# lzzcd001/MeshDiffusion

Measured on AMD Instinct MI355X. Metric: denoise steps/sec on 64^3x4 DMTet grids (sample-steps/s = n_gpus*batch*steps/wall), higher is better.
Workload: dtype f16f6 in the Winograd convs behind a GroupNorm (fp16 hi*hi MFMA + MX block-scaled e2m3 cross terms in a K-concatenated scaled MFMA at twice the e4m3 rate; operands and weights equalised per input channel by a power of two: md_wino_equaliser, after the load-time calibration from the measured operand

## Files before the change

### include/meshdiffusion_hip.h

```cpp
#ifndef MESHDIFFUSION_HIP_H
#define MESHDIFFUSION_HIP_H

#include <stdint.h>

#ifdef __cplusplus
extern "C" {
#endif

#define MD_OK 0
#define MD_ERR_BAD_ARG (-1)
#define MD_ERR_UNSUPPORTED (-2)
#define MD_ERR_NO_DEVICE (-3)

#define MD_ABI_VERSION 16

enum {
  MD_CFG_C3_128 = 0,
  MD_CFG_C3_128_K16 = 1,
  MD_CFG_C3_32 = 2,
  MD_CFG_C3_LOW = 3,
  MD_CFG_C3_S2 = 4,
  MD_CFG_G1_128 = 5,
  MD_CFG_G1_128_LOW = 6,
  MD_CFG_G1_64_LOW = 7,
// ... 86 lines not shown
                           int32_t W, void* stream);
int md_ncdhw_to_s16b(const float* x, void* out, int32_t batch, int32_t C, int32_t c_pad,
                     int64_t P, void* stream);
int md_f32b_to_ncdhw(const float* x, float* out, int32_t batch, int32_t C, int64_t P, void* stream);
int md_ncdhw_to_f32b(const float* x, float* out, int32_t batch, int32_t C, int64_t P, void* stream);
int md_s16b_to_ncdhw(const void* x, float* out, int32_t batch, int32_t C, int64_t P, void* stream);

int md_softmax_keys(const float* s, void* p, int32_t batch, int32_t n_keys, int32_t n_q,
                    void* stream);

int md_nin_f32(const float* x1, const float* x2, int32_t c1, int32_t c2, const void* wpk, const float* bias,
               float* out, int32_t batch, int32_t cout, int64_t P, int32_t n_cu, void* stream);

int64_t md_wino_operand_bytes(int32_t batch, int32_t cin, int32_t D, int32_t H, int32_t W);
int md_wino_prep(const float* x1, const float* x2, int32_t c1, int32_t c2, const float* ac, int32_t silu, int32_t ups,
                 void* t_out, int32_t batch, int32_t D, int32_t H, int32_t W, float drop_p, uint64_t drop_seed, void* stream);
int64_t md_wino_weight_bytes(int32_t cout, int32_t cin);
int md_wino_pack_weights(const float* w, void* wpk, int32_t cout, int32_t cin, int64_t s_row, int64_t s_k, int32_t flip,
                         void* stream);
int md_conv3_wino(const void* t_in, const void* wpk, float* out, const float* bias, int64_t bias_bstride,
                  const float* residual, int64_t res_bstride, double* stats, int32_t batch, int32_t cin, int32_t cout,
                  int32_t D, int32_t H, int32_t W, int32_t variant, void* stream);

int md_wino_equaliser(const float* gamma, const float* beta, const float* w, int32_t cout, int32_t cin, int64_t s_row, int64_t s_k,
                      float* eq, void* stream);
int md_wino_equaliser_measured(const float* gamma, const float* beta, const float* w, const float* a2m, int32_t cout, int32_t cin,
                               int64_t s_row, int64_t s_k, float* eq, void* stream);
int md_wino_operand_ms(const float* x1, const float* x2, int32_t c1, int32_t c2, const float* ac, int32_t silu, int32_t batch, int64_t P,
                       float* ms, void* stream);
int md_wino_prep_f8(const float* x1, const float* x2, int32_t c1, int32_t c2, const float* ac, int32_t silu, int32_t ups,
                    const float* eq, void* t_out, int32_t batch, int32_t D, int32_t H, int32_t W, void* stream);
int64_t md_wino_weight_bytes_f8(int32_t cout, int32_t cin);
int md_wino_pack_weights_f8(const float* w, const float* eq, void* wpk, int32_t cout, int32_t cin, int64_t s_row, int64_t s_k, void* stream);
int md_conv3_wino_f8(const void* t_in, const void* wpk, float* out, const float* bias, int64_t bias_bstride,
                     const float* residual, int64_t res_bstride, double* stats, int32_t batch, int32_t cin, int32_t cout,
                     int32_t D, int32_t H, int32_t W, void* stream);
int md_absmax(const float* x, int64_t n, uint32_t* amax_bits, void* stream);
int md_wino_prep_dual_f6(const float* x, int32_t c, void* t_out, void* u_out, float* sums, float tscale, const uint32_t* amax_bits,
                         int32_t batch, int32_t D, int32_t H, int32_t W, void* stream);
int md_conv3_wino_f6_scaled(const void* t_in, const void* wpk, float* out, const float* bias, int64_t bias_bstride,
                            const float* residual, int64_t res_bstride, double* stats, int32_t batch, int32_t cin, int32_t cout,
                            int32_t D, int32_t H, int32_t W, float out_scale, const uint32_t* amax_bits, void* stream);

int md_wino_prep_f6(const float* x1, const float* x2, int32_t c1, int32_t c2, const float* ac, int32_t silu, int32_t ups,
                    const float* eq, void* t_out, int32_t batch, int32_t D, int32_t H, int32_t W, void* stream);
int md_wino_pack_weights_f6(const float* w, const float* eq, void* wpk, int32_t cout, int32_t cin, int64_t s_row, int64_t s_k, void* stream);
int md_conv3_wino_f6(const void* t_in, const void* wpk, float* out, const float* bias, int64_t bias_bstride,
                     const float* residual, int64_t res_bstride, double* stats, int32_t batch, int32_t cin, int32_t cout,
                     int32_t D, int32_t H, int32_t W, void* stream);

int md_wino_prep_f6_nin(const float* x1, const float* x2, int32_t c1, int32_t c2, const float* ac, int32_t silu, const float* eq,
                        void* t_out, const void* wpk, const float* bias, float* res, int32_t batch, int32_t D, int32_t H, int32_t W,
                        int32_t n_cu, void* stream);

#define MD_WINO_FMT_BF16X3 0
#define MD_WINO_FMT_F16F8 1
#define MD_WINO_FMT_F16F6 2
int md_wino_prep_upsdh(int32_t fmt, const float* x1, const float* x2, int32_t c1, int32_t c2, const float* ac, int32_t silu,
                       const float* eq, void* t_out, int32_t batch, int32_t D, int32_t H, int32_t W, void* stream);
int md_conv3_wino_upsdh(int32_t fmt, const void* t_in, const void* wpk, float* out, const float* bias, int64_t bias_bstride,
                        const float* residual, int64_t res_bstride, double* stats, int32_t batch, int32_t cin, int32_t cout,
                        int32_t D, int32_t H, int32_t W, void* stream);

int md_conv3_stem(const void* x16, const void* wpk, float* out, const float* bias, const float* residual, double* stats,
                  int32_t batch, int32_t cout, int32_t D, int32_t H, int32_t W, void* stream);

int md_conv3_head(const float* x, const float* ac, const void* wpk, float* y, int32_t batch, int32_t cin, int32_t rows_alloc,
                  int32_t D, int32_t H, int32_t W, void* stream);

enum { MD_PACK_WPK = 0, MD_PACK_WINO = 1, MD_PACK_WINO_F6 = 2 };
typedef struct MdPackJob {
  const float* w;
  void* out;
  int64_t s_row, s_k, s_tap, n_items, block0;
  int32_t rows, kdim, taps, nt, kc, prec, flip, kind;
} MdPackJob;
int md_pack_batch(const MdPackJob* jobs_dev, int32_t n_jobs, int64_t total_blocks, int32_t tiled, void* stream);

int md_conv3_s2(const float* x, const void* wpk, float* out, const float* bias, int64_t bias_bstride, double* stats,
                int32_t batch, int32_t cin, int32_t rows, int32_t rows_alloc, int32_t D, int32_t H, int32_t W, void* stream);

int md_wino_prep_v2(const float* x1, const float* x2, int32_t c1, int32_t c2, const float* ac, int32_t silu, int32_t ups,
                    void* t_out, int32_t batch, int32_t D, int32_t H, int32_t W, float drop_p, uint64_t drop_seed, void* stream);

int md_wino_prep_dual(const float* x1, const float* x2, int32_t c1, int32_t c2, const float* ac, int32_t silu, int32_t ups,
                      void* t_out, void* u_out, float* sums, int32_t batch, int32_t D, int32_t H, int32_t W, float drop_p,
                      uint64_t drop_seed, void* stream);

int md_attn_fwd(const void* qk, const void* vT, void* out, const float* bias_v, int32_t batch, int32_t C,
                int32_t N, float scale, void* stream);

int md_ancestral_step(const float* x, const float* eps, const float* z, const float* mask,
                      const float* coef, float* x_out, float* x_mean_out, int32_t batch,
                      int32_t C, int64_t P, void* stream);
int md_ddim_step(const double* x, const float* eps, const float* mask, const double* coef, const float* partial,
                 const float* pmask, int32_t ch, double* x_out, double* x0_out, float* x_f32, int32_t batch,
                 int32_t C, int64_t P, void* stream);
#define MD_LANGEVIN_SLABS 64
#define MD_CORRECTOR_LANGEVIN 0
#define MD_CORRECTOR_ALD 1
#define MD_SDE_REVERSE_DIFFUSION 0
#define MD_SDE_EULER_MARUYAMA 1
int md_langevin_norms(const float* eps, const float* z, int32_t batch, int32_t C, int64_t P, double* slabs, void* stream);
int md_langevin_step(const float* x, const float* eps, const float* z, const float* mask, const float* coef,
                     const double* slabs, float snr, int32_t mode, float* x_out, float* x_mean_out, float* step_out,
                     int32_t batch, int32_t C, int64_t P, void* stream);
// ... 159 lines not shown
```

### meshdiffusion_amd/_lib.py

```python
import ctypes as C
import os

_HERE = os.path.dirname(os.path.abspath(__file__))
LIB_PATH = os.environ.get("MD_LIB") or os.path.join(_HERE, "libmeshdiffusion_hip.so")

(CFG_C3_128, CFG_C3_128_K16, CFG_C3_32, CFG_C3_LOW, CFG_C3_S2, CFG_G1_128, CFG_G1_128_LOW, CFG_G1_64_LOW,
 CFG_C3_128_V2, CFG_C3_128_SW, CFG_C3_128_PIPE) = range(11)
(CFG_C3_128_FAST, CFG_C5_128_K16, CFG_C5_32_K16, CFG_C3_128_W4, CFG_C3X_32, CFG_C5X_32_K16, CFG_C3X_128_K16, CFG_C5X_128,
 CFG_G1_128_N128) = range(14, 23)
OUT_F32B, OUT_S16B, OUT_NCDHW = 0, 1, 2
PREC_BF16X3, PREC_FP16X2 = 0, 1
A_PACKED, A_S16B = 0, 1
B_S16B, B_F32B_GN = 0, 1
CORRECTOR_LANGEVIN, CORRECTOR_ALD = 0, 1
SDE_REVERSE_DIFFUSION, SDE_EULER_MARUYAMA = 0, 1
LANGEVIN_SLABS = 64

CFG_NT_KC = {
    CFG_C3_128: (128, 32), CFG_C3_128_K16: (128, 16), CFG_C3_32: (32, 32), CFG_C3_LOW: (128, 32),
    CFG_C3_S2: (128, 32), CFG_G1_128: (128, 32), CFG_G1_128_LOW: (128, 32), CFG_G1_64_LOW: (64, 32),
    CFG_C3_128_V2: (128, 32), CFG_C3_128_SW: (128, 32), CFG_C3_128_PIPE: (128, 32),
    CFG_C3_128_FAST: (128, 32), CFG_C5_128_K16: (128, 16), CFG_C5_32_K16: (32, 16), CFG_C3_128_W4: (128, 32), CFG_C3X_32: (32, 32), CFG_C5X_32_K16: (32, 16), CFG_C3X_128_K16: (128, 16), CFG_C5X_128: (128, 32), CFG_G1_128_N128: (128, 32),
}
ABLATION_CFG_NT_KC = {c: (128, 32) for c in (101, 102, 103, 104, 105, 111, 113, 114, 116, 117, 118, 122)}
# ... 16 lines not shown
    _fields_ = [
        ("w", C.c_void_p), ("out", C.c_void_p), ("s_row", C.c_int64), ("s_k", C.c_int64), ("s_tap", C.c_int64),
        ("n_items", C.c_int64), ("block0", C.c_int64), ("rows", C.c_int32), ("kdim", C.c_int32), ("taps", C.c_int32),
        ("nt", C.c_int32), ("kc", C.c_int32), ("prec", C.c_int32), ("flip", C.c_int32), ("kind", C.c_int32),
    ]


PACK_WPK, PACK_WINO, PACK_WINO_F6 = 0, 1, 2
WINO_FMT = {False: 0, "f8": 1, "f6": 2}
ABI_VERSION = 16
_P, _I32, _I64, _F, _U64 = C.c_void_p, C.c_int32, C.c_int64, C.c_float, C.c_uint64

SIGNATURES = {
    "md_abi_version": (C.c_int, []),
    "md_device_count": (C.c_int, []),
    "md_gemm_conv": (C.c_int, [C.POINTER(MdGemmConvArgs), _P]),
    "md_gemm_conv_partial_bytes": (_I64, [C.POINTER(MdGemmConvArgs)]),
    "md_gemm_conv_cfg_info": (C.c_int, [_I32] + [C.POINTER(C.c_int32)] * 6),
    "md_pack_weights": (C.c_int, [_P, _P, _I32, _I32, _I32, _I64, _I64, _I64, _I32, _I32, _I32, _P]),
    "md_packed_weight_bytes": (_I64, [_I32, _I32, _I32, _I32, _I32]),
    "md_gn_stats": (C.c_int, [_P, _P, _I32, _I32, _I64, _I32, _I32, _P]),
    "md_gn_finalize": (C.c_int, [_P, _P, _P, _P, _I32, _I32, _I32, _I64, _F, _P, _P]),
    "md_gn_apply": (C.c_int, [_P, _P, _P, _P, _I32, _I32, _I64, _I32, _I32, _I32, _I32, _F, _U64, _P]),
    "md_dropout_scale": (C.c_int, [_P, _I32, _I32, _I64, _I32, _I32, _F, _U64, _P]),
    "md_zero": (C.c_int, [_P, _I64, _P]),
    "md_timestep_embedding": (C.c_int, [_P, _P, _I32, _I32, _P]),
    "md_linear": (C.c_int, [_P, _P, _P, _P, _I32, _I32, _I32, _I32, _P]),
    "md_ncdhw_to_s16b_xfold": (C.c_int, [_P, _P, _I32, _I32, _I32, _I32, _I32, _I32, _I32, _P]),
    "md_fold_dx": (C.c_int, [_P, _P, _P, _I32, _I32, _I32, _I32, _I32, _I32, _I32, _P]),
    "md_ncdhw_to_s16b": (C.c_int, [_P, _P, _I32, _I32, _I32, _I64, _P]),
    "md_f32b_to_ncdhw": (C.c_int, [_P, _P, _I32, _I32, _I64, _P]),
    "md_ncdhw_to_f32b": (C.c_int, [_P, _P, _I32, _I32, _I64, _P]),
    "md_s16b_to_ncdhw": (C.c_int, [_P, _P, _I32, _I32, _I64, _P]),
    "md_nin_f32": (C.c_int, [_P, _P, _I32, _I32, _P, _P, _P, _I32, _I32, _I64, _I32, _P]),
    "md_wino_operand_bytes": (_I64, [_I32, _I32, _I32, _I32, _I32]),
    "md_wino_prep": (C.c_int, [_P, _P, _I32, _I32, _P, _I32, _I32, _P, _I32, _I32, _I32, _I32, _F, _U64, _P]),
    "md_wino_weight_bytes": (_I64, [_I32, _I32]),
    "md_wino_pack_weights": (C.c_int, [_P, _P, _I32, _I32, _I64, _I64, _I32, _P]),
    "md_conv3_wino": (C.c_int, [_P, _P, _P, _P, _I64, _P, _I64, _P, _I32, _I32, _I32, _I32, _I32, _I32, _I32, _P]),
    "md_wino_equaliser": (C.c_int, [_P, _P, _P, _I32, _I32, _I64, _I64, _P, _P]),
    "md_wino_equaliser_measured": (C.c_int, [_P, _P, _P, _P, _I32, _I32, _I64, _I64, _P, _P]),
    "md_wino_operand_ms": (C.c_int, [_P, _P, _I32, _I32, _P, _I32, _I32, _I64, _P, _P]),
    "md_wino_prep_f8": (C.c_int, [_P, _P, _I32, _I32, _P, _I32, _I32, _P, _P, _I32, _I32, _I32, _I32, _P]),
    "md_wino_weight_bytes_f8": (_I64, [_I32, _I32]),
    "md_wino_pack_weights_f8": (C.c_int, [_P, _P, _P, _I32, _I32, _I64, _I64, _P]),
    "md_conv3_wino_f8": (C.c_int, [_P, _P, _P, _P, _I64, _P, _I64, _P, _I32, _I32, _I32, _I32, _I32, _I32, _P]),
    "md_absmax": (C.c_int, [_P, _I64, _P, _P]),
    "md_wino_prep_dual_f6": (C.c_int, [_P, _I32, _P, _P, _P, _F, _P, _I32, _I32, _I32, _I32, _P]),
    "md_conv3_wino_f6_scaled": (C.c_int, [_P, _P, _P, _P, _I64, _P, _I64, _P, _I32, _I32, _I32, _I32, _I32, _I32, _F, _P, _P]),
    "md_wino_prep_f6": (C.c_int, [_P, _P, _I32, _I32, _P, _I32, _I32, _P, _P, _I32, _I32, _I32, _I32, _P]),
    "md_wino_pack_weights_f6": (C.c_int, [_P, _P, _P, _I32, _I32, _I64, _I64, _P]),
    "md_conv3_wino_f6": (C.c_int, [_P, _P, _P, _P, _I64, _P, _I64, _P, _I32, _I32, _I32, _I32, _I32, _I32, _P]),
    "md_wino_prep_f6_nin": (C.c_int, [_P, _P, _I32, _I32, _P, _I32, _P, _P, _P, _P, _P, _I32, _I32, _I32, _I32, _I32, _P]),
    "md_wino_prep_upsdh": (C.c_int, [_I32, _P, _P, _I32, _I32, _P, _I32, _P, _P, _I32, _I32, _I32, _I32, _P]),
    "md_conv3_wino_upsdh": (C.c_int, [_I32, _P, _P, _P, _P, _I64, _P, _I64, _P, _I32, _I32, _I32, _I32, _I32, _I32, _P]),
    "md_conv3_stem": (C.c_int, [_P, _P, _P, _P, _P, _P, _I32, _I32, _I32, _I32, _I32, _P]),
    "md_conv3_head": (C.c_int, [_P, _P, _P, _P, _I32, _I32, _I32, _I32, _I32, _I32, _P]),
    "md_pack_batch": (C.c_int, [_P, _I32, _I64, _I32, _P]),
    "md_conv3_s2": (C.c_int, [_P, _P, _P, _P, _I64, _P, _I32, _I32, _I32, _I32, _I32, _I32, _I32, _P]),
    "md_wino_prep_v2": (C.c_int, [_P, _P, _I32, _I32, _P, _I32, _I32, _P, _I32, _I32, _I32, _I32, _F, _U64, _P]),
    "md_wino_prep_dual": (C.c_int, [_P, _P, _I32, _I32, _P, _I32, _I32, _P, _P, _P, _I32, _I32, _I32, _I32, _F, _U64, _P]),
    "md_wgrad_wino_workspace_bytes": (_I64, [_I32, _I32, _I32]),
    "md_wgrad_wino": (C.c_int, [_P, _P, _P, _P, _I64, _I32, _I32, _I32, _I32, _I32, _I32, _I32, _I64, _I64, _I64, _P]),
    "md_wgrad_nin_workspace_bytes": (_I64, [_I32, _I32, _I32]),
    "md_wgrad_nin": (C.c_int, [_P, _P, _P, _P, _I64, _I32, _I32, _I32, _I64, _I32, _I64, _I64, _P]),
    "md_attn_fwd": (C.c_int, [_P, _P, _P, _P, _I32, _I32, _I32, _F, _P]),
    "md_softmax_keys": (C.c_int, [_P, _P, _I32, _I32, _I32, _P]),
    "md_ancestral_step": (C.c_int, [_P, _P, _P, _P, _P, _P, _P, _I32, _I32, _I64, _P]),
    "md_ddim_step": (C.c_int, [_P, _P, _P, _P, _P, _P, _I32, _P, _P, _P, _I32, _I32, _I64, _P]),
    "md_langevin_norms": (C.c_int, [_P, _P, _I32, _I32, _I64, _P, _P]),
    "md_langevin_step": (C.c_int, [_P, _P, _P, _P, _P, _P, _F, _I32, _P, _P, _P, _I32, _I32, _I64, _P]),
    "md_sde_step": (C.c_int, [_P, _P, _P, _P, _P, _I32, _P, _P, _I32, _I32, _I64, _P]),
    "md_inpaint_blend": (C.c_int, [_P, _P, _P, _P, _I32, _I32, _I32, _I64, _I64, _P]),
    "md_inpaint_renoise": (C.c_int, [_P, _P, _P, _P, _P, _P, _I32, _I32, _I32, _I64, _P]),
    "md_ddpm_perturb": (C.c_int, [_P, _P, _P, _P, _P, _I32, _I32, _I64, _P]),
    "md_masked_sq_err": (C.c_int, [_P, _P, _P, _P, _P, _F, _I32, _I32, _I64, _P]),
    "md_grad_sqnorm": (C.c_int, [_P, _I64, _P, _P]),
    "md_adam_ema_step": (C.c_int, [_P, _P, _P, _P, _P, _I64, _F, _F, _F, _F, _F, _I32, _F, _P, _F, _P]),
    "md_pb16_bytes": (_I64, [_I32, _I32, _I32, _I32, _I32, _I32, _I32]),
    "md_to_pb16": (C.c_int, [_P, _P, _I32, _I32, _I32, _I32, _I32, _I32, _I32, _I32, _I32, _I32, _I32, _I32, _I32, _P]),
    "md_wgrad_finish": (C.c_int, [_P, _P, _I32, _I32, _I32, _I32, _I32, _I64, _I64, _I64, _P]),
    "md_wgrad_workspace_bytes": (_I64, [_I32, _I32, _I32, _I32]),
    "md_wgrad": (C.c_int, [_P, _P, _P, _P, _I64, _I32, _I32, _I32, _I32, _I32, _I32, _I32, _I32, _I32, _I32, _I32, _I64, _I64,
                           _I64, _P]),
    "md_gn_bwd_stats": (C.c_int, [_P, _P, _P, _P, _I32, _I32, _I64, _I32, _I32, _I32, _I32, _F, _U64, _P]),
    "md_gn_bwd_finalize": (C.c_int, [_P, _P, _P, _P, _P, _P, _I32, _I32, _I32, _I64, _P]),
    "md_gn_bwd_apply": (C.c_int, [_P, _P, _P, _P, _P, _I32, _I32, _I64, _I32, _I32, _I32, _I32, _I32, _F, _U64, _P, _P, _P, _P]),
    "md_channel_sums": (C.c_int, [_P, _P, _I32, _I32, _I64, _P]),
    "md_s16b_transpose": (C.c_int, [_P, _P, _I32, _I32, _I32, _P]),
    "md_softmax_keys_bwd": (C.c_int, [_P, _P, _P, _I32, _I32, _I32, _F, _P]),
    "md_grad_resample": (C.c_int, [_P, _P, _I32, _I32, _I32, _I32, _I32, _I32, _I32, _P]),
    "md_marching_tets_workspace_bytes": (_I64, [_I32, _I32, _I32]),
    "md_vertex_normals": (C.c_int, [_P, _P, _I64, _I64, _P, _P, _P]),
    "md_marching_tets": (C.c_int, [_P, _P, _P, _P, _P, _I32, _I32, _I32, _I32, _P, _P, _P, _P, _P, _I64, _P]),
    "md_marching_tets_bwd": (C.c_int, [_P, _P, _P, _P, _P, _P, _P, _P, _I32, _I32, _I32, _P, _P, _P]),
    "md_sdf_reg_loss": (C.c_int, [_P, _P, _I32, _I32, _P, _P, _P, _P]),
    "md_sdf_reg_loss_bwd": (C.c_int, [_P, _P, _P, _P, _P, _P, _I32, _I32, _P, _P]),
    "md_nn_sided_workspace_bytes": (_I64, [_I32, _I32, _I32]),
    "md_nn_sided": (C.c_int, [_P, _P, _I32, _I32, _I32, _I32, _P, _P, _P, _I64, _P]),
    "md_chamfer_bwd": (C.c_int, [_P, _P, _P, _P, _P, _P, _P, _P, _I32, _I32, _I32, _F, _F, _P, _P, _P, _P]),
    "md_face_areas": (C.c_int, [_P, _P, _I32, _I32, _I32, _P, _P]),
    "md_sample_points": (C.c_int, [_P, _P, _P, _P, _P, _P, _P, _I32, _I32, _I32, _I32, _P, _P, _P, _P]),
    "md_sample_points_bwd": (C.c_int, [_P, _P, _P, _P, _I32, _I32, _I32, _P, _P]),
    "md_raster_bin_count": (C.c_int, [_P, _P, _I32, _I32, _I32, _I32, _I32, _P, _P]),
    "md_raster_bin_emit": (C.c_int, [_P, _P, _P, _I32, _I32, _I32, _I32, _I32, _I64, _P, _P, _P]),
    "md_raster_tiles": (C.c_int, [_P, _P, _P, _P, _I32, _I32, _I32, _I32, _I32, _P, _P, _P]),
# ... 84 lines not shown
```

### meshdiffusion_amd/csrc/block_pass.hip

```cpp
#include "md_common.h"
#include "md_prep_f6.h"

namespace {
constexpr int BP_ROWS = 128, BP_WAVES = 8, BP_THREADS = BP_WAVES * 64, BP_TILE = BP_WAVES * 32;

__device__ __forceinline__ uint64_t bp_uniform(const void* p) {
  const uint64_t v = (uint64_t)p;
  const uint32_t lo = __builtin_amdgcn_readfirstlane((uint32_t)v), hi = __builtin_amdgcn_readfirstlane((uint32_t)(v >> 32));
  return ((uint64_t)hi << 32) | lo;
}
typedef uint32_t bp_u32x4 __attribute__((ext_vector_type(4)));
typedef __attribute__((address_space(1))) const bp_u32x4* bp_gload_t;
typedef __attribute__((address_space(1))) bp_u32x4* bp_gstore_u_t;
typedef __attribute__((address_space(1))) f32x4* bp_gstore_t;
__device__ __forceinline__ uint4 bp_load(uint64_t base, uint32_t off) { return __builtin_bit_cast(uint4, *(bp_gload_t)(base + off)); }
__device__ __forceinline__ void bp_store(uint64_t base, uint32_t off, f32x4 v) { *(bp_gstore_t)(base + off) = v; }
__device__ __forceinline__ void bp_store(uint64_t base, uint32_t off, uint4 v) {
  *(bp_gstore_u_t)(base + off) = __builtin_bit_cast(bp_u32x4, v);
}
__device__ __forceinline__ float bp_pull(int addr, float v) {
  return __builtin_bit_cast(float, __builtin_amdgcn_ds_bpermute(addr, __builtin_bit_cast(int, v)));
}
}

template <int KSTEPS, bool NIN>
__global__ __launch_bounds__(BP_THREADS) void md_block_pass_kernel(const uint4* __restrict__ x1, const uint4* __restrict__ x2, int split8,
                                                                   int c1, int c2, const float* __restrict__ ac, int silu,
                                                                   const float* __restrict__ eq, uint4* __restrict__ T,
                                                                   const uint4* __restrict__ wpk, const float* __restrict__ bias,
                                                                   float* __restrict__ res, int64_t P, int W, int n_tiles,
                                                                   int tiles_per_sample) {
  constexpr int GS = 4;
  constexpr int NG = KSTEPS / GS;
  constexpr int K = KSTEPS * 16;
  __shared__ __attribute__((aligned(16))) uint4 wl[NIN ? (KSTEPS / 2) * 4 * 2 * BP_ROWS : 1];
  __shared__ __attribute__((aligned(16))) float acl[BP_WAVES][2 * K];
  __shared__ __attribute__((aligned(16))) float eql[K];
  const int tid = threadIdx.x, lane = tid & 63;
  const int wid = __builtin_amdgcn_readfirstlane(tid >> 6);
  const int j = lane & 31, h = lane >> 5;
  if constexpr (NIN) {
    for (int i = tid; i < (KSTEPS / 2) * 1024; i += BP_THREADS) wl[i] = wpk[i];
  }
  if (eq != nullptr && tid < K) eql[tid] = eq[tid];
  __syncthreads();
  const unsigned char* wb = (const unsigned char*)wl;
  const int64_t Ph = P >> 1;

  const int xr = (wid * 32 + j) & (W - 1);
  const bool has_l = xr > 0, has_r = xr < W - 1;
  const bool first = j == 0, last = j == 31;
  const bool take_l = has_l && !first, take_r = has_r && !last, use_h = (first && has_l) || (last && has_r);
  const bool odd = j & 1;
  const int a_l = ((lane - 1) & 63) * 4, a_r = ((lane + 1) & 63) * 4;
  const int hk = (lane >> 3) & 3, hh = (lane >> 2) & 1, hend = (lane >> 1) & 1, hq = lane & 1;
  const bool seg_l = ((wid * 32) & (W - 1)) != 0, seg_r = ((wid * 32 + 32) & (W - 1)) != 0;
  const bool hload = lane < 32 && (hend ? seg_r : seg_l);
  const int a_h = (4 * h + 2 * (last ? 1 : 0)) * 4;

  uint4 s0[2 * GS], s1[2 * GS], g0 = make_uint4(0, 0, 0, 0), g1 = g0;
  const uint32_t loff = (uint32_t)(((int64_t)h * P + wid * 32 + j) * 32);
  auto issue = [&](uint4 (&st)[2 * GS], uint4& hreg, int t, int g) {
    const int b = t / tiles_per_sample;
    const int64_t p0 = (int64_t)(t - b * tiles_per_sample) * BP_TILE;
#pragma unroll
    for (int k = 0; k < GS; ++k) {
      const int ks = g * GS + k;
      const uint64_t ub = bp_uniform((2 * ks < split8) ? (const char*)x1 + (((int64_t)b * (c1 >> 3) + 2 * ks) * P + p0) * 32
                                                    : (const char*)x2 + (((int64_t)b * (c2 >> 3) + (2 * ks - split8)) * P + p0) * 32);
      st[2 * k] = bp_load(ub, loff);
      st[2 * k + 1] = bp_load(ub, loff + 16);
    }
    if (hload) {
      const int cg = 2 * (g * GS + hk) + hh;
      const char* src = cg < split8 ? (const char*)x1 + ((int64_t)b * (c1 >> 3) + cg) * P * 32
                                    : (const char*)x2 + ((int64_t)b * (c2 >> 3) + (cg - split8)) * P * 32;
      hreg = *(const uint4*)(src + (p0 + wid * 32 + (hend ? 32 : -1)) * 32 + hq * 16);
    }
  };
  f32x16 acc[NIN ? 4 : 1];
  auto step = [&](int ks, const uint4& r0, const uint4& r1) {
    uint32_t hw[4], lw[4];
    md_split2(__uint_as_float(r0.x), __uint_as_float(r0.y), hw[0], lw[0]);
    md_split2(__uint_as_float(r0.z), __uint_as_float(r0.w), hw[1], lw[1]);
    md_split2(__uint_as_float(r1.x), __uint_as_float(r1.y), hw[2], lw[2]);
    md_split2(__uint_as_float(r1.z), __uint_as_float(r1.w), hw[3], lw[3]);
    const bf16x8 bhi = __builtin_bit_cast(bf16x8, make_uint4(hw[0], hw[1], hw[2], hw[3]));
    const bf16x8 blo = __builtin_bit_cast(bf16x8, make_uint4(lw[0], lw[1], lw[2], lw[3]));
    const unsigned char* wt = wb + (ks >> 1) * 16384 + (((2 * (ks & 1) + h) * 2) * BP_ROWS + j) * 16;
#pragma unroll
    for (int rt = 0; rt < (NIN ? 4 : 0); ++rt) {
      const bf16x8 ahi = *(const bf16x8*)(wt + rt * 32 * 16);
      const bf16x8 alo = *(const bf16x8*)(wt + (BP_ROWS + rt * 32) * 16);
      acc[rt] = __builtin_amdgcn_mfma_f32_32x32x16_bf16(alo, bhi, acc[rt], 0, 0, 0);
      acc[rt] = __builtin_amdgcn_mfma_f32_32x32x16_bf16(ahi, blo, acc[rt], 0, 0, 0);
      acc[rt] = __builtin_amdgcn_mfma_f32_32x32x16_bf16(ahi, bhi, acc[rt], 0, 0, 0);
    }
    __builtin_amdgcn_sched_barrier(0);
  };
  const float* aw = acl[wid];
  auto activate4 = [&](float (&y)[4], int ch) {
    if (ac != nullptr) {
      const f32x4 p0 = *(const f32x4*)(aw + 2 * ch), p1 = *(const f32x4*)(aw + 2 * ch + 4);
      y[0] = md_prep_act(y[0], p0[0], p0[1], silu);
      y[1] = md_prep_act(y[1], p0[2], p0[3], silu);
      y[2] = md_prep_act(y[2], p1[0], p1[1], silu);
      y[3] = md_prep_act(y[3], p1[2], p1[3], silu);
    }
    if (eq != nullptr) {
      const f32x4 e4 = *(const f32x4*)(eql + ch);
#pragma unroll
      for (int e = 0; e < 4; ++e) y[e] = md_prep_eq(y[e], e4[e]);
    }
  };
  auto prep = [&](int ks, int k, const uint4& r0, const uint4& r1, const float (&hv)[4], uint64_t tb) {
    float ya[4] = {__uint_as_float(r0.x), __uint_as_float(r0.y), __uint_as_float(r0.z), __uint_as_float(r0.w)};
    float yb[4] = {__uint_as_float(r1.x), __uint_as_float(r1.y), __uint_as_float(r1.z), __uint_as_float(r1.w)};
    activate4(ya, 16 * ks + 8 * h);
    activate4(yb, 16 * ks + 8 * h + 4);
    float fa[8], fb[8];
#pragma unroll
    for (int e = 0; e < 8; ++e) {
      float own = e < 4 ? ya[e] : yb[e - 4];
      asm("" : "+v"(own));
      const float hl = bp_pull(a_h + (8 * k + (e >> 2)) * 4, hv[e & 3]);
      const float edge = use_h ? hl : 0.f;
      const float pl = bp_pull(a_l, own), pr = bp_pull(a_r, own);
      const float l = take_l ? pl : edge, r = take_r ? pr : edge;
      const float lr = md_wino_bt(0, l, 0.f, r, 0.f);
      const float f1 = md_wino_bt(1, 0.f, own, r, 0.f);
      const float f2 = md_wino_bt(2, 0.f, l, own, 0.f);
      fa[e] = odd ? f2 : lr;
      fb[e] = odd ? lr : f1;
    }
    __builtin_amdgcn_sched_barrier(0);
    float t[16];
#pragma unroll
    for (int e = 0; e < 8; ++e) {
      const auto sw = __builtin_amdgcn_permlane32_swap(__builtin_bit_cast(uint32_t, fa[e]), __builtin_bit_cast(uint32_t, fb[e]), false, false);
      t[e] = __uint_as_float(sw[0]);
      t[8 + e] = __uint_as_float(sw[1]);
    }
    uint4 h0, h1, q0, q1;
    md_split_f16f6(t, false, 0, h0, h1, q0, q1);
    const uint32_t voff = (uint32_t)(((int64_t)(2 * (2 * (j & 1) + h)) * Ph + (j >> 1)) * 16);
    const uint32_t plane = (uint32_t)(Ph * 16), group = (uint32_t)(8 * Ph * 16);
    bp_store(tb, voff, h0);
    bp_store(tb, voff + plane, q0);
    bp_store(tb, voff + group, h1);
    bp_store(tb, voff + group + plane, q1);
    __builtin_amdgcn_sched_barrier(0);
  };
  auto consume = [&](uint4 (&st)[2 * GS], const uint4& hreg, int g, int b, int64_t p0) {
    float hv[4] = {__uint_as_float(hreg.x), __uint_as_float(hreg.y), __uint_as_float(hreg.z), __uint_as_float(hreg.w)};
    activate4(hv, 16 * (g * GS + hk) + 8 * hh + 4 * hq);
#pragma unroll
    for (int k = 0; k < GS; ++k) {
      const int ks = g * GS + k;
      if constexpr (NIN) step(ks, st[2 * k], st[2 * k + 1]);
      const uint64_t tb = bp_uniform((const char*)T + ((((int64_t)b * (K / 8) + 2 * ks) * 8) * Ph + ((p0 + wid * 32) >> 1)) * 16);
      prep(ks, k, st[2 * k], st[2 * k + 1], hv, tb);
    }
  };

  int t = blockIdx.x, cur_b = -1;
  if (t < n_tiles) { issue(s0, g0, t, 0); issue(s1, g1, t, 1); }
  for (; t < n_tiles; t += gridDim.x) {
    const int tn = t + gridDim.x;
    const int b = t / tiles_per_sample;
    const int64_t p0 = (int64_t)(t - b * tiles_per_sample) * BP_TILE;
    if (ac != nullptr && b != cur_b) {
      cur_b = b;
      const f32x4* src = (const f32x4*)(ac + (int64_t)b * 2 * K);
      for (int i = 0; i < 2 * K / 4 / 64; ++i) *(f32x4*)(acl[wid] + (i * 64 + lane) * 4) = src[i * 64 + lane];
      __builtin_amdgcn_fence(__ATOMIC_RELEASE, "wavefront");
      __builtin_amdgcn_wave_barrier();
      __builtin_amdgcn_fence(__ATOMIC_ACQUIRE, "wavefront");
    }
    if constexpr (NIN) {
#pragma unroll
      for (int rt = 0; rt < 4; ++rt) {
#pragma unroll
        for (int r = 0; r < 16; ++r) acc[rt][r] = 0.f;
      }
    }
#pragma unroll 1
    for (int gc = 0; gc < NG; gc += 2) {
      int g = gc;
      asm volatile("" : "+s"(g));
      const bool same = g + 2 < NG;
      const bool more = same || tn < n_tiles;
      const int ti = same ? t : tn, gi = same ? g + 2 : g + 2 - NG;
      consume(s0, g0, g, b, p0);
      if (more) issue(s0, g0, ti, gi);
      __builtin_amdgcn_sched_barrier(0);
      consume(s1, g1, g + 1, b, p0);
      if (more) issue(s1, g1, ti, gi + 1);
      __builtin_amdgcn_sched_barrier(0);
    }
    if constexpr (NIN) {
      const uint32_t soff = (uint32_t)((wid * 32 + j) * 32 + 16 * h);
#pragma unroll
      for (int rt = 0; rt < 4; ++rt)
#pragma unroll
        for (int q = 0; q < 4; ++q) {
          const int row = rt * 32 + 8 * q + 4 * h;
          const f32x4 bv = *(const f32x4*)(bias + row);
          f32x4 o4;
#pragma unroll
          for (int e = 0; e < 4; ++e) o4[e] = acc[rt][q * 4 + e] + bv[e];
          const uint64_t ub = bp_uniform((char*)res + (((int64_t)b * (BP_ROWS / 8) + rt * 4 + q) * P + p0) * 32);
          bp_store(ub, soff, o4);
        }
    }
  }
}

template <int KSTEPS, bool NIN>
static void bp_launch(int blocks, hipStream_t st, const float* x1, const float* x2, int c1, int c2, const float* ac, int silu, const float* eq,
                      void* T, const void* wpk, const float* bias, float* res, int64_t P, int W, int n_tiles) {
  hipLaunchKernelGGL((md_block_pass_kernel<KSTEPS, NIN>), dim3((unsigned)blocks), dim3(BP_THREADS), 0, st, (const uint4*)x1, (const uint4*)x2,
                     c1 >> 3, c1, c2, ac, silu, eq, (uint4*)T, (const uint4*)wpk, bias, res, P, W, n_tiles, (int)(P / BP_TILE));
}

extern "C" int md_wino_prep_f6_nin(const float* x1, const float* x2, int32_t c1, int32_t c2, const float* ac, int32_t silu, const float* eq,
                                   void* t_out, const void* wpk, const float* bias, float* res, int32_t batch, int32_t D, int32_t H,
                                   int32_t W, int32_t n_cu, void* stream) {
  if (!x1 || !t_out || batch <= 0 || c1 <= 0 || c2 < 0 || (c1 & 15) || (c2 & 15) || (c2 > 0 && !x2)) return MD_ERR_BAD_ARG;
  if (silu && !ac) return MD_ERR_BAD_ARG;
  if (D <= 0 || H <= 0 || W <= 0 || (W & 1)) return MD_ERR_BAD_ARG;
  if (wpk && (!bias || !res)) return MD_ERR_BAD_ARG;
  const int64_t P = (int64_t)D * H * W;
  if ((BP_TILE % W) || (P % BP_TILE)) return MD_ERR_UNSUPPORTED;
  const int K = c1 + c2;
  if (K != 128 && K != 256) return MD_ERR_UNSUPPORTED;
  if (P > ((int64_t)1 << 25)) return MD_ERR_UNSUPPORTED;
  const int64_t n_tiles64 = (int64_t)batch * (P / BP_TILE);
  if (n_tiles64 > 0x7fffffff) return MD_ERR_UNSUPPORTED;
  const int n_tiles = (int)n_tiles64;
  int blocks = n_cu > 0 ? n_cu : 256;
  if (blocks > n_tiles) blocks = n_tiles;
  hipStream_t st = (hipStream_t)stream;
  MD_HIP_CLEAR_ERROR();
  if (wpk) {
    if (K == 256) bp_launch<16, true>(blocks, st, x1, x2, c1, c2, ac, silu, eq, t_out, wpk, bias, res, P, W, n_tiles);
    else bp_launch<8, true>(blocks, st, x1, x2, c1, c2, ac, silu, eq, t_out, wpk, bias, res, P, W, n_tiles);
  } else {
    if (K == 256) bp_launch<16, false>(blocks, st, x1, x2, c1, c2, ac, silu, eq, t_out, wpk, bias, res, P, W, n_tiles);
    else bp_launch<8, false>(blocks, st, x1, x2, c1, c2, ac, silu, eq, t_out, wpk, bias, res, P, W, n_tiles);
  }
  MD_HIP_CHECK_LAUNCH();
  return MD_OK;
}
```

### meshdiffusion_amd/csrc/md_common.h

```cpp
#pragma once
#include <hip/hip_runtime.h>
#include <hip/hip_fp16.h>
#include <stdint.h>
#include "meshdiffusion_hip.h"

typedef __attribute__((ext_vector_type(8))) short bf16x8;
typedef __attribute__((ext_vector_type(16))) float f32x16;
typedef __attribute__((ext_vector_type(4))) float f32x4;

#define MD_HIP_CLEAR_ERROR() (void)hipGetLastError()
#define MD_HIP_CHECK_LAUNCH()                      \
  do {                                             \
    hipError_t e__ = hipGetLastError();            \
    if (e__ != hipSuccess) return (int)e__;        \
  } while (0)

__device__ __forceinline__ uint32_t md_f2bf(float f) {
  uint32_t u = __float_as_uint(f);
  u += 0x7FFFu + ((u >> 16) & 1u);
  return u >> 16;
}
__device__ __forceinline__ float md_bf2f(uint32_t h) { return __uint_as_float(h << 16); }

__device__ __forceinline__ void md_split(float x, uint32_t& hi, uint32_t& lo) {
// ... 2 lines not shown
}

typedef __bf16 md_bf16x2 __attribute__((ext_vector_type(2)));
typedef float md_f32x2 __attribute__((ext_vector_type(2)));
__device__ __forceinline__ void md_split2(float x0, float x1, uint32_t& hi, uint32_t& lo) {
  const md_f32x2 y = {x0, x1};
  hi = __builtin_bit_cast(uint32_t, __builtin_convertvector(y, md_bf16x2));
  const md_f32x2 hf = {__uint_as_float(hi << 16), __uint_as_float(hi & 0xffff0000u)};
  lo = __builtin_bit_cast(uint32_t, __builtin_convertvector(y - hf, md_bf16x2));
}

typedef _Float16 f16x8 __attribute__((ext_vector_type(8)));
__device__ __forceinline__ uint32_t md_f2h(float f) {
  f = fminf(fmaxf(f, -65504.f), 65504.f);
  return (uint32_t)__half_as_ushort(__float2half_rn(f));
}
__device__ __forceinline__ float md_h2f(uint32_t h) { return __half2float(__ushort_as_half((unsigned short)h)); }
__device__ __forceinline__ void md_split_f16(float x, uint32_t& hi, uint32_t& lo) {
  hi = md_f2h(x);
  lo = md_f2h(x - md_h2f(hi));
}

__device__ __forceinline__ float md_clamp448(float x) { return __builtin_amdgcn_fmed3f(x, -448.f, 448.f); }
__device__ __forceinline__ float md_sat_f16_finite(float x) { return __builtin_isfinite(x) ? __builtin_amdgcn_fmed3f(x, -65504.f, 65504.f) : x; }
__device__ __forceinline__ uint32_t md_f16f8_pair(float a, float b, float& la, float& lb) {
  const _Float16 ha = (_Float16)md_sat_f16_finite(a), hb = (_Float16)md_sat_f16_finite(b);
  la = (a - (float)ha) * 2048.f;
  lb = (b - (float)hb) * 2048.f;
  return (uint32_t)__builtin_bit_cast(unsigned short, ha) | ((uint32_t)__builtin_bit_cast(unsigned short, hb) << 16);
}
__device__ __forceinline__ uint32_t md_e4m3x4(float a, float b, float c, float d) {
  int v = __builtin_amdgcn_cvt_pk_fp8_f32(md_clamp448(a), md_clamp448(b), 0, false);
  return (uint32_t)__builtin_amdgcn_cvt_pk_fp8_f32(md_clamp448(c), md_clamp448(d), v, true);
}
__device__ __forceinline__ void md_split_f16f8(const float (&t)[8], uint4& hi, uint32_t (&q)[2], uint32_t (&ql)[2]) {
  float l[8];
  hi.x = md_f16f8_pair(t[0], t[1], l[0], l[1]);
  hi.y = md_f16f8_pair(t[2], t[3], l[2], l[3]);
  hi.z = md_f16f8_pair(t[4], t[5], l[4], l[5]);
  hi.w = md_f16f8_pair(t[6], t[7], l[6], l[7]);
  q[0] = md_e4m3x4(t[0], t[1], t[2], t[3]);
  q[1] = md_e4m3x4(t[4], t[5], t[6], t[7]);
  ql[0] = md_e4m3x4(l[0], l[1], l[2], l[3]);
  ql[1] = md_e4m3x4(l[4], l[5], l[6], l[7]);
}

typedef float md_f32x16 __attribute__((ext_vector_type(16)));
typedef uint32_t md_u32x6 __attribute__((ext_vector_type(6)));
__device__ __forceinline__ md_u32x6 md_cvt_2xpk16_fp6(md_f32x16 a, md_f32x16 b) {
  md_u32x6 r;
  asm("v_cvt_scalef32_2xpk16_fp6_f32 %0, %1, %2, 1.0" : "=&v"(r) : "v"(a), "v"(b));
  return r;
}
__device__ __forceinline__ void md_split_f16f6(const float (&t)[16], bool lo_first, int scale_bias, uint4& hi0, uint4& hi1, uint4& r0,
                                               uint4& r1) {
  float l[16];
  uint32_t hw[8];
#pragma unroll
  for (int i = 0; i < 8; ++i) hw[i] = md_f16f8_pair(t[2 * i], t[2 * i + 1], l[2 * i], l[2 * i + 1]);
  hi0 = make_uint4(hw[0], hw[1], hw[2], hw[3]);
  hi1 = make_uint4(hw[4], hw[5], hw[6], hw[7]);
  float m = 0.f;
#pragma unroll
  for (int i = 0; i < 16; ++i) m = fmaxf(m, fmaxf(fabsf(t[i]), fabsf(l[i])));
  int eb = (int)(__float_as_uint(m) >> 23);
  eb = eb < 20 ? 20 : eb;
  const float inv = __uint_as_float((uint32_t)(256 - eb) << 23);
  md_f32x16 a, b;
#pragma unroll
  for (int i = 0; i < 16; ++i) {
    a[i] = (lo_first ? l[i] : t[i]) * inv;
    b[i] = (lo_first ? t[i] : l[i]) * inv;
  }
  const md_u32x6 c = md_cvt_2xpk16_fp6(a, b);
  r0 = make_uint4(c[0], c[1], c[2], c[3]);
  r1 = make_uint4(c[4], c[5], (uint32_t)(eb - 2 + scale_bias), 0u);
}

__device__ __forceinline__ uint64_t md_drop_bits(uint64_t seed, uint64_t q) {
  uint64_t z = seed + (q + 1) * 0x9E3779B97F4A7C15ull;
  z = (z ^ (z >> 30)) * 0xBF58476D1CE4E5B9ull;
  z = (z ^ (z >> 27)) * 0x94D049BB133111EBull;
  return z ^ (z >> 31);
}
__device__ __forceinline__ bool md_drop_keep(uint64_t bits, int e, uint32_t thr16) {
  return (uint32_t)((bits >> (16 * e)) & 0xFFFFu) >= thr16;
}
static inline uint32_t md_drop_thr16(float p) {
  const float t = p * 65536.0f + 0.5f;
  return t <= 0.f ? 0u : (t >= 65535.f ? 65535u : (uint32_t)t);
}

__device__ __forceinline__ float md_silu(float x) { return x / (1.0f + expf(-x)); }

__device__ __forceinline__ float md_wave_sum(float v) {
#pragma unroll
  for (int o = 32; o > 0; o >>= 1) v += __shfl_xor(v, o, 64);
  return v;
}
__device__ __forceinline__ int md_dgrad_lift_log2(uint32_t amax_bits) {
  const float amax = __uint_as_float(amax_bits);
  if (!(amax > 0.f) || !(amax < 3e38f)) return 0;
  const int k = 4 - ilogbf(amax);
  return k < -60 ? -60 : (k > 60 ? 60 : k);
}
__device__ __forceinline__ float md_wave_max(float v) {
#pragma unroll
  for (int o = 32; o > 0; o >>= 1) v = fmaxf(v, __shfl_xor(v, o, 64));
  return v;
}
```

### meshdiffusion_amd/csrc/md_prep_f6.h

```cpp
#pragma once
#include "md_common.h"

__device__ __forceinline__ float md_prep_act(float t, float a, float c, int silu) {
  t = t * a + c;
  if (silu) t = t * __builtin_amdgcn_rcpf(1.0f + __builtin_amdgcn_exp2f(t * -1.4426950408889634f));
  return t;
}

__device__ __forceinline__ float md_prep_eq(float y, float s) {
#pragma clang fp contract(off)
  return y * s;
}

__device__ __forceinline__ float md_wino_bt(int f, float d0, float d1, float d2, float d3) {
#pragma clang fp contract(off)
  return f == 0 ? d0 - d2 : f == 1 ? d1 + d2 : f == 2 ? d2 - d1 : d1 - d3;
}
```

Before: 112.6.

## Replace bpermute neighbor exchange with LDS staging in block-pass Winograd prep

The Winograd input-transform prep in the fused block-pass kernel no longer gathers left, right and halo neighbours with ds_bpermute plus a permlane32 swap. Each wave now writes its activated values and halo into a per-wave LDS scratch with zero slots, orders the accesses with wave-scoped fences, and reads two operands per lane. The B^T row is then computed as a single vector add with a sign-flip mask. Separately, the f16/fp6 split uses a cheaper unsaturated f16 conversion and falls back to the saturating path only when a wave sees non-finite values; address arithmetic for loads and stores is hoisted into running offsets. This adds LDS footprint, which may lower occupancy, and a host helper that exposes the exchange map for testing.

```diff
diff --git a/include/meshdiffusion_hip.h b/include/meshdiffusion_hip.h
--- a/include/meshdiffusion_hip.h
+++ b/include/meshdiffusion_hip.h
@@ -162,6 +162,7 @@
 int md_wino_prep_f6_nin(const float* x1, const float* x2, int32_t c1, int32_t c2, const float* ac, int32_t silu, const float* eq,
                         void* t_out, const void* wpk, const float* bias, float* res, int32_t batch, int32_t D, int32_t H, int32_t W,
                         int32_t n_cu, void* stream);
+int md_block_pass_exchange_map(int32_t W, int32_t wid, int32_t* map, int32_t* geom);
 
 #define MD_WINO_FMT_BF16X3 0
 #define MD_WINO_FMT_F16F8 1
diff --git a/meshdiffusion_amd/_lib.py b/meshdiffusion_amd/_lib.py
--- a/meshdiffusion_amd/_lib.py
+++ b/meshdiffusion_amd/_lib.py
@@ -92,6 +92,7 @@
     "md_wino_pack_weights_f6": (C.c_int, [_P, _P, _P, _I32, _I32, _I64, _I64, _P]),
     "md_conv3_wino_f6": (C.c_int, [_P, _P, _P, _P, _I64, _P, _I64, _P, _I32, _I32, _I32, _I32, _I32, _I32, _P]),
     "md_wino_prep_f6_nin": (C.c_int, [_P, _P, _I32, _I32, _P, _I32, _P, _P, _P, _P, _P, _I32, _I32, _I32, _I32, _I32, _P]),
+    "md_block_pass_exchange_map": (C.c_int, [_I32, _I32, _P, _P]),
     "md_wino_prep_upsdh": (C.c_int, [_I32, _P, _P, _I32, _I32, _P, _I32, _P, _P, _I32, _I32, _I32, _I32, _P]),
     "md_conv3_wino_upsdh": (C.c_int, [_I32, _P, _P, _P, _P, _I64, _P, _I64, _P, _I32, _I32, _I32, _I32, _I32, _I32, _P]),
     "md_conv3_stem": (C.c_int, [_P, _P, _P, _P, _P, _P, _I32, _I32, _I32, _I32, _I32, _P]),
diff --git a/meshdiffusion_amd/csrc/block_pass.hip b/meshdiffusion_amd/csrc/block_pass.hip
--- a/meshdiffusion_amd/csrc/block_pass.hip
+++ b/meshdiffusion_amd/csrc/block_pass.hip
@@ -18,8 +18,39 @@
 __device__ __forceinline__ void bp_store(uint64_t base, uint32_t off, uint4 v) {
   *(bp_gstore_u_t)(base + off) = __builtin_bit_cast(bp_u32x4, v);
 }
-__device__ __forceinline__ float bp_pull(int addr, float v) {
-  return __builtin_bit_cast(float, __builtin_amdgcn_ds_bpermute(addr, __builtin_bit_cast(int, v)));
+
+constexpr int BP_XSLOTS = 34 + 16, BP_XPLANE = BP_XSLOTS * 16, BP_XBYTES = 2 * BP_XPLANE;
+__host__ __device__ inline int bp_x_write(int j, int h) { return h * BP_XPLANE + (j + 1) * 16; }
+__host__ __device__ inline int bp_x_halo(int hh, int hend) { return hh * BP_XPLANE + (hend ? 33 : 0) * 16; }
+struct bp_holder {
+  int hk, hh, hend, hq;
+  bool seg_l, seg_r, loads;
+};
+__host__ __device__ inline bp_holder bp_x_holder(int lane, int seg0, int W) {
+  bp_holder o;
+  o.hk = (lane >> 3) & 3; o.hh = (lane >> 2) & 1; o.hend = (lane >> 1) & 1; o.hq = lane & 1;
+  o.seg_l = (seg0 & (W - 1)) != 0; o.seg_r = ((seg0 + 32) & (W - 1)) != 0;
+  o.loads = lane < 32 && (o.hend ? o.seg_r : o.seg_l);
+  return o;
+}
+__host__ __device__ inline bool bp_x_halo_writes(const bp_holder& o, int lane, int k, int q) {
+  return (o.seg_l || o.seg_r) && (lane & 0x39) == 8 * k + q;
+}
+__host__ __device__ inline int bp_x_freq(int lane) { return (0x2130 >> ((lane >> 4) * 4)) & 3; }
+__host__ __device__ inline int bp_x_zero(int slot) { return 34 + ((slot - 34) & 15); }
+__host__ __device__ inline void bp_x_reads(int lane, int seg0, int W, int& ra, int& rb) {
+  const int p = lane & 15, f = bp_x_freq(lane);
+  int sa = 2 * p + (f == 0 ? 0 : f == 2 ? 2 : 1), sb = 2 * p + (f == 3 ? 3 : f == 2 ? 1 : 2);
+  const int xe = (seg0 + 2 * p) & (W - 1);
+  if (f == 0 && xe == 0) sa = bp_x_zero(sa);
+  if (f == 3 && xe == W - 2) sb = bp_x_zero(sb);
+  ra = sa * 16;
+  rb = sb * 16;
+}
+__device__ __forceinline__ void bp_x_order() {
+  __builtin_amdgcn_fence(__ATOMIC_RELEASE, "wavefront");
+  __builtin_amdgcn_wave_barrier();
+  __builtin_amdgcn_fence(__ATOMIC_ACQUIRE, "wavefront");
 }
 }
 
@@ -36,6 +67,7 @@
   __shared__ __attribute__((aligned(16))) uint4 wl[NIN ? (KSTEPS / 2) * 4 * 2 * BP_ROWS : 1];
   __shared__ __attribute__((aligned(16))) float acl[BP_WAVES][2 * K];
   __shared__ __attribute__((aligned(16))) float eql[K];
+  __shared__ __attribute__((aligned(16))) unsigned char xl[BP_WAVES][BP_XBYTES];
   const int tid = threadIdx.x, lane = tid & 63;
   const int wid = __builtin_amdgcn_readfirstlane(tid >> 6);
   const int j = lane & 31, h = lane >> 5;
@@ -47,35 +79,42 @@
   const unsigned char* wb = (const unsigned char*)wl;
   const int64_t Ph = P >> 1;
 
-  const int xr = (wid * 32 + j) & (W - 1);
-  const bool has_l = xr > 0, has_r = xr < W - 1;
-  const bool first = j == 0, last = j == 31;
-  const bool take_l = has_l && !first, take_r = has_r && !last, use_h = (first && has_l) || (last && has_r);
-  const bool odd = j & 1;
-  const int a_l = ((lane - 1) & 63) * 4, a_r = ((lane + 1) & 63) * 4;
-  const int hk = (lane >> 3) & 3, hh = (lane >> 2) & 1, hend = (lane >> 1) & 1, hq = lane & 1;
-  const bool seg_l = ((wid * 32) & (W - 1)) != 0, seg_r = ((wid * 32 + 32) & (W - 1)) != 0;
-  const bool hload = lane < 32 && (hend ? seg_r : seg_l);
-  const int a_h = (4 * h + 2 * (last ? 1 : 0)) * 4;
+  const bp_holder ho = bp_x_holder(lane, wid * 32, W);
+  const int hk = ho.hk, hh = ho.hh, hend = ho.hend, hq = ho.hq;
+  const bool hload = ho.loads;
+  unsigned char* const xw = xl[wid];
+  unsigned char* const x_wr = xw + bp_x_write(j, h);
+  unsigned char* const x_hw = xw + bp_x_halo(hh, hend);
+  const int xp = lane & 15, xf = bp_x_freq(lane);
+  int ra, rb;
+  bp_x_reads(lane, wid * 32, W, ra, rb);
+  const unsigned char* const x_ra = xw + ra;
+  const unsigned char* const x_rb = xw + rb;
+  const uint32_t x_flip = xf == 1 ? 0u : 0x80000000u;
+  if (lane < 32) *(f32x4*)(xw + (lane >> 4) * BP_XPLANE + (34 + (lane & 15)) * 16) = f32x4{0.f, 0.f, 0.f, 0.f};
+  bp_x_order();
 
   uint4 s0[2 * GS], s1[2 * GS], g0 = make_uint4(0, 0, 0, 0), g1 = g0;
   const uint32_t loff = (uint32_t)(((int64_t)h * P + wid * 32 + j) * 32);
   auto issue = [&](uint4 (&st)[2 * GS], uint4& hreg, int t, int g) {
     const int b = t / tiles_per_sample;
     const int64_t p0 = (int64_t)(t - b * tiles_per_sample) * BP_TILE;
+    const uint64_t xstep = (uint64_t)P * 64;
+    const uint64_t b1 = (uint64_t)x1 + (uint64_t)(((int64_t)b * (c1 >> 3) * P + p0) * 32);
+    const uint64_t b2 = (uint64_t)x2 + (uint64_t)((((int64_t)b * (c2 >> 3) - split8) * P + p0) * 32);
+    uint64_t o = (uint64_t)(g * GS) * xstep;
 #pragma unroll
     for (int k = 0; k < GS; ++k) {
       const int ks = g * GS + k;
-      const uint64_t ub = bp_uniform((2 * ks < split8) ? (const char*)x1 + (((int64_t)b * (c1 >> 3) + 2 * ks) * P + p0) * 32
-                                                    : (const char*)x2 + (((int64_t)b * (c2 >> 3) + (2 * ks - split8)) * P + p0) * 32);
+      const uint64_t ub = bp_uniform((const void*)(((2 * ks < split8) ? b1 : b2) + o));
+      o += xstep;
       st[2 * k] = bp_load(ub, loff);
       st[2 * k + 1] = bp_load(ub, loff + 16);
     }
     if (hload) {
       const int cg = 2 * (g * GS + hk) + hh;
-      const char* src = cg < split8 ? (const char*)x1 + ((int64_t)b * (c1 >> 3) + cg) * P * 32
-                                    : (const char*)x2 + ((int64_t)b * (c2 >> 3) + (cg - split8)) * P * 32;
-      hreg = *(const uint4*)(src + (p0 + wid * 32 + (hend ? 32 : -1)) * 32 + hq * 16);
+      const uint64_t src = (cg < split8 ? b1 : b2) + (uint64_t)((int64_t)cg * P * 32);
+      hreg = *(const uint4*)(src + (int64_t)((wid * 32 + (hend ? 32 : -1)) * 32 + hq * 16));
     }
   };
   f32x16 acc[NIN ? 4 : 1];
@@ -113,37 +152,48 @@
       for (int e = 0; e < 4; ++e) y[e] = md_prep_eq(y[e], e4[e]);
     }
   };
+  auto activate8 = [&](float (&y)[8], int ch) {
+    if (ac != nullptr) {
+#pragma unroll
+      for (int e = 0; e < 8; e += 2) {
+        const f32x4 p = *(const f32x4*)(aw + 2 * (ch + e));
+        y[e] = md_prep_act(y[e], p[0], p[1], silu);
+        y[e + 1] = md_prep_act(y[e + 1], p[2], p[3], silu);
+      }
+    }
+    if (eq != nullptr) {
+#pragma unroll
+      for (int e = 0; e < 8; ++e) y[e] = md_prep_eq(y[e], (e < 4 ? *(const f32x4*)(eql + ch) : *(const f32x4*)(eql + ch + 4))[e & 3]);
+    }
+  };
   auto prep = [&](int ks, int k, const uint4& r0, const uint4& r1, const float (&hv)[4], uint64_t tb) {
-    float ya[4] = {__uint_as_float(r0.x), __uint_as_float(r0.y), __uint_as_float(r0.z), __uint_as_float(r0.w)};
-    float yb[4] = {__uint_as_float(r1.x), __uint_as_float(r1.y), __uint_as_float(r1.z), __uint_as_float(r1.w)};
-    activate4(ya, 16 * ks + 8 * h);
-    activate4(yb, 16 * ks + 8 * h + 4);
-    float fa[8], fb[8];
-#pragma unroll
-    for (int e = 0; e < 8; ++e) {
-      float own = e < 4 ? ya[e] : yb[e - 4];
-      asm("" : "+v"(own));
-      const float hl = bp_pull(a_h + (8 * k + (e >> 2)) * 4, hv[e & 3]);
-      const float edge = use_h ? hl : 0.f;
-      const float pl = bp_pull(a_l, own), pr = bp_pull(a_r, own);
-      const float l = take_l ? pl : edge, r = take_r ? pr : edge;
-      const float lr = md_wino_bt(0, l, 0.f, r, 0.f);
-      const float f1 = md_wino_bt(1, 0.f, own, r, 0.f);
-      const float f2 = md_wino_bt(2, 0.f, l, own, 0.f);
-      fa[e] = odd ? f2 : lr;
-      fb[e] = odd ? lr : f1;
+    float y[8] = {__uint_as_float(r0.x), __uint_as_float(r0.y), __uint_as_float(r0.z), __uint_as_float(r0.w),
+                  __uint_as_float(r1.x), __uint_as_float(r1.y), __uint_as_float(r1.z), __uint_as_float(r1.w)};
+    activate8(y, 16 * ks + 8 * h);
+    float t[16];
+#pragma unroll
+    for (int q = 0; q < 2; ++q) {
+      *(f32x4*)x_wr = f32x4{y[4 * q], y[4 * q + 1], y[4 * q + 2], y[4 * q + 3]};
+      if (bp_x_halo_writes(ho, lane, k, q)) *(f32x4*)x_hw = f32x4{hv[0], hv[1], hv[2], hv[3]};
+      bp_x_order();
+      f32x4 da[2], db[2];
+#pragma unroll
+      for (int hp = 0; hp < 2; ++hp) {
+        da[hp] = *(const f32x4*)(x_ra + hp * BP_XPLANE);
+        db[hp] = *(const f32x4*)(x_rb + hp * BP_XPLANE);
+      }
+      bp_x_order();
+#pragma unroll
+      for (int hp = 0; hp < 2; ++hp) {
+        const f32x4 tv = md_wino_bt_signed(da[hp], db[hp], x_flip);
+#pragma unroll
+        for (int e = 0; e < 4; ++e) t[8 * hp + 4 * q + e] = tv[e];
+      }
     }
     __builtin_amdgcn_sched_barrier(0);
-    float t[16];
-#pragma unroll
-    for (int e = 0; e < 8; ++e) {
-      const auto sw = __builtin_amdgcn_permlane32_swap(__builtin_bit_cast(uint32_t, fa[e]), __builtin_bit_cast(uint32_t, fb[e]), false, false);
-      t[e] = __uint_as_float(sw[0]);
-      t[8 + e] = __uint_as_float(sw[1]);
-    }
     uint4 h0, h1, q0, q1;
     md_split_f16f6(t, false, 0, h0, h1, q0, q1);
-    const uint32_t voff = (uint32_t)(((int64_t)(2 * (2 * (j & 1) + h)) * Ph + (j >> 1)) * 16);
+    const uint32_t voff = (uint32_t)(((int64_t)(2 * xf) * Ph + xp) * 16);
     const uint32_t plane = (uint32_t)(Ph * 16), group = (uint32_t)(8 * Ph * 16);
     bp_store(tb, voff, h0);
     bp_store(tb, voff + plane, q0);
@@ -151,15 +201,15 @@
     bp_store(tb, voff + group + plane, q1);
     __builtin_amdgcn_sched_barrier(0);
   };
-  auto consume = [&](uint4 (&st)[2 * GS], const uint4& hreg, int g, int b, int64_t p0) {
+  auto consume = [&](uint4 (&st)[2 * GS], const uint4& hreg, int g, uint64_t tb, uint64_t tstep) {
     float hv[4] = {__uint_as_float(hreg.x), __uint_as_float(hreg.y), __uint_as_float(hreg.z), __uint_as_float(hreg.w)};
     activate4(hv, 16 * (g * GS + hk) + 8 * hh + 4 * hq);
 #pragma unroll
     for (int k = 0; k < GS; ++k) {
       const int ks = g * GS + k;
       if constexpr (NIN) step(ks, st[2 * k], st[2 * k + 1]);
-      const uint64_t tb = bp_uniform((const char*)T + ((((int64_t)b * (K / 8) + 2 * ks) * 8) * Ph + ((p0 + wid * 32) >> 1)) * 16);
-      prep(ks, k, st[2 * k], st[2 * k + 1], hv, tb);
+      prep(ks, k, st[2 * k], st[2 * k + 1], hv, bp_uniform((const void*)tb));
+      tb += tstep;
     }
   };
 
@@ -184,6 +234,8 @@
         for (int r = 0; r < 16; ++r) acc[rt][r] = 0.f;
       }
     }
+    const uint64_t tstep = (uint64_t)Ph * 256, tgroup = GS * tstep;
+    uint64_t tb = (uint64_t)T + (uint64_t)(((int64_t)b * K * Ph + ((p0 + wid * 32) >> 1)) * 16);
 #pragma unroll 1
     for (int gc = 0; gc < NG; gc += 2) {
       int g = gc;
@@ -191,10 +243,12 @@
       const bool same = g + 2 < NG;
       const bool more = same || tn < n_tiles;
       const int ti = same ? t : tn, gi = same ? g + 2 : g + 2 - NG;
-      consume(s0, g0, g, b, p0);
+      consume(s0, g0, g, tb, tstep);
+      tb += tgroup;
       if (more) issue(s0, g0, ti, gi);
       __builtin_amdgcn_sched_barrier(0);
-      consume(s1, g1, g + 1, b, p0);
+      consume(s1, g1, g + 1, tb, tstep);
+      tb += tgroup;
       if (more) issue(s1, g1, ti, gi + 1);
       __builtin_amdgcn_sched_barrier(0);
     }
@@ -252,3 +306,23 @@
   MD_HIP_CHECK_LAUNCH();
   return MD_OK;
 }
+
+extern "C" int md_block_pass_exchange_map(int32_t W, int32_t wid, int32_t* map, int32_t* geom) {
+  if (!map || !geom || W < 2 || (W & (W - 1)) || (BP_TILE % W) || wid < 0 || wid >= BP_WAVES) return MD_ERR_BAD_ARG;
+  for (int lane = 0; lane < 64; ++lane) {
+    const int j = lane & 31, h = lane >> 5;
+    const bp_holder ho = bp_x_holder(lane, wid * 32, W);
+    int ra, rb, mask = 0;
+    bp_x_reads(lane, wid * 32, W, ra, rb);
+    for (int k = 0; k < 4; ++k)
+      for (int q = 0; q < 2; ++q) mask |= bp_x_halo_writes(ho, lane, k, q) ? 1 << (2 * k + q) : 0;
+    int32_t* m = map + 14 * lane;
+    m[0] = j; m[1] = h; m[2] = bp_x_write(j, h);
+    m[3] = bp_x_halo(ho.hh, ho.hend);
+    m[4] = ho.hk; m[5] = ho.hh; m[6] = ho.hend; m[7] = ho.hq;
+    m[8] = ho.loads;
+    m[9] = lane & 15; m[10] = bp_x_freq(lane); m[11] = ra; m[12] = rb; m[13] = mask;
+  }
+  geom[0] = BP_XBYTES; geom[1] = BP_XPLANE; geom[2] = 34 * 16; geom[3] = 16;
+  return MD_OK;
+}
diff --git a/meshdiffusion_amd/csrc/md_common.h b/meshdiffusion_amd/csrc/md_common.h
--- a/meshdiffusion_amd/csrc/md_common.h
+++ b/meshdiffusion_amd/csrc/md_common.h
@@ -78,17 +78,35 @@
   asm("v_cvt_scalef32_2xpk16_fp6_f32 %0, %1, %2, 1.0" : "=&v"(r) : "v"(a), "v"(b));
   return r;
 }
+typedef _Float16 md_f16x2 __attribute__((ext_vector_type(2)));
+template <bool SAT>
+__device__ __forceinline__ float md_f16f6_planes(const float (&t)[16], float (&l)[16], uint32_t (&hw)[8]) {
+#pragma unroll
+  for (int i = 0; i < 8; ++i) {
+    if constexpr (SAT) {
+      hw[i] = md_f16f8_pair(t[2 * i], t[2 * i + 1], l[2 * i], l[2 * i + 1]);
+    } else {
+      const md_f32x2 tv = {t[2 * i], t[2 * i + 1]};
+      const md_f16x2 hv = __builtin_convertvector(tv, md_f16x2);
+      const md_f32x2 lv = (tv - __builtin_convertvector(hv, md_f32x2)) * 2048.f;
+      l[2 * i] = lv[0];
+      l[2 * i + 1] = lv[1];
+      hw[i] = __builtin_bit_cast(uint32_t, hv);
+    }
+  }
+  float m = 0.f;
+#pragma unroll
+  for (int i = 0; i < 16; ++i) m = fmaxf(fmaxf(m, fabsf(t[i])), fabsf(l[i]));
+  return m;
+}
 __device__ __forceinline__ void md_split_f16f6(const float (&t)[16], bool lo_first, int scale_bias, uint4& hi0, uint4& hi1, uint4& r0,
                                                uint4& r1) {
   float l[16];
   uint32_t hw[8];
-#pragma unroll
-  for (int i = 0; i < 8; ++i) hw[i] = md_f16f8_pair(t[2 * i], t[2 * i + 1], l[2 * i], l[2 * i + 1]);
+  float m = md_f16f6_planes<false>(t, l, hw);
+  if (__builtin_expect(__builtin_amdgcn_ballot_w64(!(m < __builtin_inff())) != 0, 0)) m = md_f16f6_planes<true>(t, l, hw);
   hi0 = make_uint4(hw[0], hw[1], hw[2], hw[3]);
   hi1 = make_uint4(hw[4], hw[5], hw[6], hw[7]);
-  float m = 0.f;
-#pragma unroll
-  for (int i = 0; i < 16; ++i) m = fmaxf(m, fmaxf(fabsf(t[i]), fabsf(l[i])));
   int eb = (int)(__float_as_uint(m) >> 23);
   eb = eb < 20 ? 20 : eb;
   const float inv = __uint_as_float((uint32_t)(256 - eb) << 23);
diff --git a/meshdiffusion_amd/csrc/md_prep_f6.h b/meshdiffusion_amd/csrc/md_prep_f6.h
--- a/meshdiffusion_amd/csrc/md_prep_f6.h
+++ b/meshdiffusion_amd/csrc/md_prep_f6.h
@@ -16,3 +16,11 @@
 #pragma clang fp contract(off)
   return f == 0 ? d0 - d2 : f == 1 ? d1 + d2 : f == 2 ? d2 - d1 : d1 - d3;
 }
+
+typedef float md_f32x4v __attribute__((ext_vector_type(4)));
+typedef uint32_t md_u32x4v __attribute__((ext_vector_type(4)));
+__device__ __forceinline__ md_f32x4v md_wino_bt_signed(md_f32x4v a, md_f32x4v b, uint32_t flip) {
+#pragma clang fp contract(off)
+  const md_u32x4v fv = {flip, flip, flip, flip};
+  return a + __builtin_bit_cast(md_f32x4v, __builtin_bit_cast(md_u32x4v, b) ^ fv);
+}
```

Measured after the change: 113.7 (median of 6 runs). Within noise of the previous version (+1.0%).
